# buggyyang/CDC_compression

Measured on AMD Instinct MI355X. Metric: decoded images/sec at 256x256, 500-step x-param, higher is better.
Workload: dtype f32 (f16x2 split products)

## Files before the change

cdc_compression_amd/csrc/conv_args.h:

```cpp
#pragma once
#include <stdint.h>

namespace cdc {

constexpr int kWaveSize = 64;
constexpr int kXS = 20;

struct ConvArgs {
    const float *src0, *src1;
    long long src0_bs, src1_bs;
    int uf_c, uf_pad;
    unsigned uf_magic;
    int C0, Cin;
    int H, W;
    const float *ln_mean, *ln_rstd;
    const float *ln_g, *ln_b;
    const float *wp;
    long long w_bs, w_zs;
    const unsigned short *wsp;
    long long wsp_zs;
    long long wsp_bs;
    float acc_scale;
    int tg;
    int ipw, B;
// ... 17 lines not shown
    float relu_slope;
    const float *shift;
    int shift_bs;
    const float *resid;
    long long resid_bs, resid_cs;
    const float *res3_w, *res3_x;
    long long res3_bs;
    float *stat_mean, *stat_rstd;
    int ksplit, nzz;
    int xcd_remap;
    int zfold;
    long long out_ks;
    void *out_pf;
    long long pf_bs, pf_ps;
    int pf_ys, pf_xs, pf_zoff[4];
    int pf_only;
    int *fault;
#ifdef CDC_TIMELINE
    unsigned long long *tl;
#endif
};

struct PfArgs {
    const void *src0, *src1;
    long long src0_bs, src1_bs;
    int C0, Cin;
    int H, W;
    const void *w;
    long long w_zs;
    int KH, KW, nz;
    int stride;
    int tz;
    int pad_y[4], pad_x[4];
    int nchunk, COP, Cout;
    float acc_scale;
    int ring;
    int n_iter;
    float *out;
    long long out_bs, out_cs;
    int out_ys, out_xs, out_zoff[4];
    void *out_pf;
    long long pf_bs, pf_ps;
    int pf_ys, pf_xs, pf_zoff[4];
    int Ho, Wo;
    int lognbw, tiles_x, tiles_y, B;
    int xcd_remap;
    const float *bias, *pre_add, *ep_g, *ep_b;
    int pre_c4;
    float eps;
    int relu;
    float relu_slope;
    const float *shift;
    int shift_bs;
    const float *resid;
    long long resid_bs, resid_cs;
    const float *resid1;
    long long resid1_bs;
    int resid_c0;
    const void *resid_pf;
    long long rpf_bs, rpf_ps;
    int rpf_ys, rpf_zoff;
    float *stat_mean, *stat_rstd;
    const float *res3_w, *res3_x;
    long long res3_bs;
    const float *x0, *x1;
    long long x0_bs, x1_bs;
    const float *pre_mean, *pre_rstd;
    long long w_bs;
    int lin;
    int dbg;
    int *fault;
#ifdef CDC_TIMELINE
    unsigned long long *tl;
#endif
};

constexpr int kPfXS = 12;

struct ConvPlan {
    int MB, NPW, WN;
    int groups;
    int KC, nchunk;
    int lognbw, tiles_x, tiles_y, PH, PW;
    int xvec, xshift[4];
    size_t lds_bytes;
    int lnmode;
    int tg;
    int ipw;
    int ksplit = 1;
    int xu = 1;
    int arith = 0;
    int split;
};

}
```

cdc_compression_amd/csrc/conv_inst_p.hip:

```cpp
#include <algorithm>
#include <map>
#include <string>
#include <vector>
#include <stdlib.h>

#include "cdc_internal.h"
#include "conv_pf_kernel.h"

namespace cdc {

template <int KH, int KW>
static pf_kernel_fn pf_lookup_k(int MB, int NPW, int WM, int WP) {
    if (MB == 2 && NPW == 2 && WM == 1 && WP == 4) return conv_pf_kernel<2, 2, 1, 4, KH, KW>;
    if (MB == 2 && NPW == 2 && WM == 2 && WP == 2) return conv_pf_kernel<2, 2, 2, 2, KH, KW>;
    if (MB == 2 && NPW == 2 && WM == 2 && WP == 4) return conv_pf_kernel<2, 2, 2, 4, KH, KW>;
    if (MB == 3 && NPW == 2 && WM == 2 && WP == 4) return conv_pf_kernel<3, 2, 2, 4, KH, KW>;
    if (MB == 3 && NPW == 1 && WM == 2 && WP == 4 && KH == 3) return conv_pf_kernel<3, 1, 2, 4, KH, KW>;
    if (MB == 2 && NPW == 2 && WM == 4 && WP == 2) return conv_pf_kernel<2, 2, 4, 2, KH, KW>;
    return nullptr;
}
static pf_kernel_fn pf_lookup_s2(int MB, int NPW, int WM, int WP) {
    if (MB == 2 && NPW == 1 && WM == 1 && WP == 4) return conv_pf_kernel<2, 1, 1, 4, 3, 3, 2>;
    if (MB == 2 && NPW == 2 && WM == 2 && WP == 2) return conv_pf_kernel<2, 2, 2, 2, 3, 3, 2>;
    if (MB == 3 && NPW == 1 && WM == 2 && WP == 4) return conv_pf_kernel<3, 1, 2, 4, 3, 3, 2>;
// ... 102 lines not shown
            if (COPT != s.Cout) continue;
            const int ring = pf_ring(c.MB, c.NPW, c.WM, c.WP, 2, 2, 1, 4);
            const int tps = pf_tps(c.MB, c.NPW, c.WM, c.WP, 2, 2, 1, 4);
            const int S = (s.Cin / 16) * 16 / tps;
            if (!ring || S < ring - 1) continue;
            const double wgs = (double)((s.Wo + 31) / 32) * ((s.Ho + TH - 1) / TH) * s.B;
            const double min_wgs = dev_env("CDC_PF_TZ_MIN_WGS") ? atof(dev_env("CDC_PF_TZ_MIN_WGS")) : 128.0;
            if (wgs < min_wgs) continue;
            best = COPT;
            const size_t patch = (size_t)2 * pf_patch_units(c.NPW, c.WP, 2, 2, 1, 4) * 16, wst = (size_t)tps * pf_rows(c.MB, 4 * c.NPW) * COPT * 16;
            p->MB = c.MB; p->NPW = c.NPW; p->WM = c.WM; p->WP = c.WP;
            p->ring = ring;
            p->tiles_x = (s.Wo + 31) / 32; p->tiles_y = (s.Ho + TH - 1) / TH;
            p->groups = 1;
            p->lds_bytes = std::max(patch + ring * wst, sizeof(float) * (size_t)(4 * COPT + 2 * c.WM * c.WP * 4 * c.NPW * 32));
            break;
        }
        return best >= 0;
    }
    for (const PfCand &c : kCands) {
        if (f[0] && (c.MB != f[0] || c.NPW != f[1] || c.WM != f[2] || c.WP != f[3])) continue;
        const int COPT = c.WM * c.MB * 32, NW = c.WM * c.WP;
        if (s.Cout % COPT) continue;
        if (s.need_all_cout && COPT != s.Cout) continue;
        if (!pf_lookup(c.MB, c.NPW, c.WM, c.WP, s.KH, s.KW)) continue;
        const int TH = c.WP * c.NPW, PH = TH + s.KH - 1, PW = 32 + s.KW - 1;
        const int xsw = (4 * PH * PW + 63) / 64;
        if (xsw > 2 * kPfXS) continue;
        const int taps = s.KH * s.KW, npb = taps == 1 ? 3 : 2;
        const size_t patch = (size_t)npb * xsw * 64 * 16, wst = (size_t)pf_rows(c.MB, c.NPW) * COPT * 16;
        const int ring = pf_ring(c.MB, c.NPW, c.WM, c.WP, s.KH, s.KW);
        if (!ring) continue;
        const int S = (s.Cin / 16) * taps;
        if (S < ring - 1) continue;
        const double wgs = (double)((s.Wo + 31) / 32) * ((s.Ho + TH - 1) / TH) * s.B * (s.Cout / COPT) * s.nz;
        const double min_waves = dev_env("CDC_PF_MIN_WAVES") ? atof(dev_env("CDC_PF_MIN_WAVES")) : 256.0;
        if (wgs * NW < min_waves) continue;
        if (c.MB == 3 && c.NPW == 1 && wgs < 128.0) continue;
        const double fill = std::min(1.0, wgs * NW / 2048.0);
        const double reads = (3.0 * c.MB + 2.0 * c.NPW) / (3.0 * c.MB * c.NPW);
        const double score = fill * (1.0 - 0.35 * reads) * (s.Cout / COPT > 1 ? 0.9 : 1.0);
        if (score > best) {
            best = score;
            p->MB = c.MB; p->NPW = c.NPW; p->WM = c.WM; p->WP = c.WP;
            p->ring = ring;
            p->tiles_x = (s.Wo + 31) / 32; p->tiles_y = (s.Ho + TH - 1) / TH;
            p->groups = s.Cout / COPT;
            p->lds_bytes = std::max(patch + ring * wst, sizeof(float) * (size_t)(4 * COPT + 2 * c.WM * c.WP * c.NPW * 32));
        }
    }
    return best >= 0;
}

hipError_t pf_launch(PfArgs a, const PfPlan &p, int B, int nz, hipStream_t st) {
    if (p.pf3_epv) return pf3_launch(a, p, B, st);
    pf_kernel_fn fn = pf_lookup(p.MB, p.NPW, p.WM, p.WP, a.KH, a.KW, a.stride == 2 ? 2 : 1, a.tz == 4 ? 4 : 1);
    if (!fn) return hipErrorInvalidValue;
    if (a.tz == 4) nz = 1;
    a.lognbw = 5;
    a.dbg = 0;
    a.tiles_x = p.tiles_x; a.tiles_y = p.tiles_y; a.B = B; a.ring = p.ring;
    if (hipError_t e = ensure_dynamic_lds((const void *)fn, p.lds_bytes); e != hipSuccess) return e;
    dim3 grid((unsigned)(p.tiles_x * p.tiles_y * B), (unsigned)p.groups, (unsigned)nz);
    a.xcd_remap = (grid.x % 8 == 0 && grid.x >= 64) ? 1 : 0;
#ifdef CDC_TIMELINE
    static unsigned long long *tl_dev = nullptr;
    static std::map<std::string, int> seen;
    const size_t tl_wgs = (size_t)grid.x * grid.y * grid.z;
    char key[96];
    snprintf(key, sizeof key, "%dx%d s%d tz%d %d->%d out %dx%d", a.KH, a.KW, a.stride == 2 ? 2 : 1, a.tz == 4 ? 4 : 1, a.Cin, a.Cout, a.Ho, a.Wo);
    a.tl = nullptr;
    if (tl_wgs <= (1u << 18) && seen[key]++ < 3) {
        if (!tl_dev) hipMalloc(&tl_dev, sizeof(unsigned long long) * 16 * (1u << 18));
        hipMemsetAsync(tl_dev, 0, sizeof(unsigned long long) * 16 * tl_wgs, st);
        a.tl = tl_dev;
    }
#endif
    hipLaunchKernelGGL(fn, grid, dim3(64 * p.WM * p.WP), p.lds_bytes, st, a);
#ifdef CDC_TIMELINE
    if (a.tl) {
        hipStreamSynchronize(st);
        std::vector<unsigned long long> h(16 * tl_wgs);
        hipMemcpy(h.data(), tl_dev, h.size() * 8, hipMemcpyDeviceToHost);
        unsigned long long t0 = ~0ull, t1 = 0;
        double cat[7] = {0}, life = 0;
        std::map<unsigned long long, int> per_cu;
        std::vector<unsigned long long> starts;
        for (size_t w = 0; w < tl_wgs; ++w) {
            const unsigned long long *r = &h[w * 16];
            for (int c = 0; c < 7; ++c) cat[c] += (double)r[c];
            t0 = std::min(t0, r[7]); t1 = std::max(t1, r[8]);
            life += (double)(r[8] - r[7]);
            per_cu[(r[10] & 0xf) << 32 | (r[9] & 0xffff00)]++;
            starts.push_back(r[7]);
        }
        std::sort(starts.begin(), starts.end());
        int cu_min = 1 << 30, cu_max = 0;
        for (auto &kv : per_cu) { cu_min = std::min(cu_min, kv.second); cu_max = std::max(cu_max, kv.second); }
        static const char *names[7] = {"setup", "prologue issue", "prologue wait", "main loop", "epilogue parameters", "epilogue arithmetic", "epilogue stores"};
        fprintf(stderr, "[pf timeline] conv %s: %zu workgroups x %d threads, lds %zu; kernel span %llu cycles, mean workgroup life %.0f; %zu CUs used, %d .. %d workgroups per CU;"
                        " start of the median / last workgroup at %llu / %llu; per workgroup (wave 0):", key, tl_wgs, 64 * p.WM * p.WP, p.lds_bytes, t1 - t0, life / tl_wgs,
                per_cu.size(), cu_min, cu_max, starts[starts.size() / 2] - t0, starts.back() - t0);
        for (int c = 0; c < 7; ++c) fprintf(stderr, "  %s %.0f", names[c], cat[c] / tl_wgs);
        fprintf(stderr, "\n");
    }
#endif
    return hipGetLastError();
}

__global__ void __launch_bounds__(256) pf_pack_kernel(const float *src, long long src_bs, uint4 *dst, long long dst_bs,
                                                      int C, int H, int W) {
    const int b = blockIdx.y;
    const long long n = (long long)(C / 8) * H * W;
    const long long i = (long long)blockIdx.x * 256 + threadIdx.x;
    if (i >= n) return;
    const int x = (int)(i % W);
    const long long t = i / W;
    const int y = (int)(t % H), g = (int)(t / H);
    const float *sp = src + (size_t)b * src_bs + ((size_t)g * 8 * H + y) * W + x;
    f16x8 hv, lv;
#pragma unroll
    for (int q = 0; q < 8; ++q) {
        _Float16 h, l;
        split2h(sp[(size_t)q * H * W], h, l);
        hv[q] = h; lv[q] = l;
    }
    const long long ps = (long long)(H + 2) * (W + 2);
    uint4 *dp = dst + (size_t)b * dst_bs + (long long)g * 2 * ps + (long long)(y + 1) * (W + 2) + x + 1;
    dp[0] = __builtin_bit_cast(uint4, hv);
    dp[ps] = __builtin_bit_cast(uint4, lv);
}

hipError_t pf_pack_launch(const float *src, long long src_bs, void *dst, long long dst_bs, int C, int H, int W, int B,
                          hipStream_t st) {
    const long long n = (long long)(C / 8) * H * W;
    dim3 grid((unsigned)((n + 255) / 256), (unsigned)B);
    hipLaunchKernelGGL(pf_pack_kernel, grid, dim3(256), 0, st, src, src_bs, reinterpret_cast<uint4 *>(dst), dst_bs, C, H, W);
    return hipGetLastError();
}

__global__ void __launch_bounds__(256) c4_pack_kernel(const float *src, long long src_bs, float4 *dst, int C, long long HW) {
    const int b = blockIdx.y;
    const long long n = (long long)(C / 4) * HW;
    const long long i = (long long)blockIdx.x * 256 + threadIdx.x;
    if (i >= n) return;
    const long long pix = i % HW, g = i / HW;
    const float *sp = src + (size_t)b * src_bs + (size_t)g * 4 * HW + pix;
    dst[(size_t)b * n + i] = make_float4(sp[0], sp[HW], sp[2 * HW], sp[3 * HW]);
}

hipError_t c4_pack_launch(const float *src, long long src_bs, float *dst, int C, long long HW, int B, hipStream_t st) {
    const long long n = (long long)(C / 4) * HW;
    dim3 grid((unsigned)((n + 255) / 256), (unsigned)B);
    hipLaunchKernelGGL(c4_pack_kernel, grid, dim3(256), 0, st, src, src_bs, reinterpret_cast<float4 *>(dst), C, HW);
// ... 28 lines not shown
```

cdc_compression_amd/csrc/conv_pf_kernel.h:

```cpp
#pragma once
#include <type_traits>

#include "conv_split_kernel.h"

namespace cdc {


#ifndef CDC_DMA_WAIT_MARGIN
#define CDC_DMA_WAIT_MARGIN 1
#endif
#ifdef CDC_DMA_WAIT_ALL
constexpr int kVmWaitMask = 0;
#else
constexpr int kVmWaitMask = ~0;
#endif
template <int N> __device__ __forceinline__ void vm_wait() { asm volatile("s_waitcnt vmcnt(%0)" ::"n"(N & kVmWaitMask) : "memory"); }

__device__ __forceinline__ void dma16(unsigned voff, const void *sbase, unsigned lds_byte) {
    asm volatile("s_mov_b32 m0, %2\n\ts_nop 0\n\tglobal_load_lds_dwordx4 %0, %1" ::"v"(voff), "s"(sbase), "s"(lds_byte)
                 : "memory");
}

template <int N, class F> __device__ __forceinline__ void static_for(F &&f) {
    if constexpr (N > 0) {
        static_for<N - 1>(f);
        f(std::integral_constant<int, N - 1>{});
    }
}

__host__ __device__ constexpr bool pf_acc2(int MB, int NPW) { return MB * NPW <= 4; }
__host__ __device__ constexpr int pf_rows(int MB, int NPW) { return pf_acc2(MB, NPW) ? 4 : 6; }
__host__ __device__ constexpr int pf_patch_units(int NPW, int WP, int KH, int KW, int STR = 1, int TZ = 1) {
    return TZ == 4 ? ((4 * (WP * NPW + 2) * 34 + 63) / 64) * 64 : ((4 * ((WP * NPW - 1) * STR + KH) * (31 * STR + KW) + 63) / 64) * 64;
}
__host__ __device__ constexpr int pf_uf_stage_floats(int NPW, int WP) { return ((3 * (WP * NPW + 6) * 38 + 63) / 64) * 64; }
#ifndef CDC_PF_S2_NPB
#define CDC_PF_S2_NPB 2
#endif
__host__ __device__ constexpr int pf_patch_bufs(int KH, int KW, int STR = 1) { return STR == 2 ? CDC_PF_S2_NPB : (KH * KW == 1 ? 3 : 2); }
__host__ __device__ constexpr int pf_ring_tps(int MB, int NPW, int WM, int WP, int KH, int KW, int STR, int tps, int TZ = 1) {
    const size_t budget = ((WM * WP == 8 || STR == 2) ? 156 * 1024 : 80 * 1024) - ((KH == 7 && KW == 1) ? pf_uf_stage_floats(NPW, WP) * 4 : 0);
    const size_t patch = (size_t)pf_patch_bufs(KH, KW, STR) * pf_patch_units(NPW, WP, KH, KW, STR, TZ) * 16;
    const size_t wst = (size_t)tps * pf_rows(MB, TZ * NPW) * WM * MB * 32 * 16;
#ifndef CDC_PF_RING_MAX
#define CDC_PF_RING_MAX 5
#endif
    for (int r = CDC_PF_RING_MAX; r >= 3; --r)
        if (patch + r * wst <= budget) return r;
    return 0;
}
#ifndef CDC_PF_S2_TPS
#define CDC_PF_S2_TPS 3
#endif
#ifndef CDC_PF_TZ_MINB
#define CDC_PF_TZ_MINB 2
#endif
#ifndef CDC_PF_TZ_TPS
#define CDC_PF_TZ_TPS 2
#endif
__host__ __device__ constexpr int pf_tps(int MB, int NPW, int WM, int WP, int KH, int KW, int STR = 1, int TZ = 1) {
    if (TZ == 4) return (CDC_PF_TZ_TPS > 1 && pf_ring_tps(MB, NPW, WM, WP, KH, KW, STR, CDC_PF_TZ_TPS, TZ) >= 3) ? CDC_PF_TZ_TPS : 1;
    return (STR == 2 && CDC_PF_S2_TPS > 1 && pf_ring_tps(MB, NPW, WM, WP, KH, KW, STR, CDC_PF_S2_TPS) >= 3) ? CDC_PF_S2_TPS : 1;
}
__host__ __device__ constexpr int pf_ring(int MB, int NPW, int WM, int WP, int KH, int KW, int STR = 1, int TZ = 1) {
    return pf_ring_tps(MB, NPW, WM, WP, KH, KW, STR, pf_tps(MB, NPW, WM, WP, KH, KW, STR, TZ), TZ);
}
#ifndef CDC_PF_ABLATE
#define CDC_PF_ABLATE 0
#endif

template <int MB, int NPW, int WM, int WP, int KH, int KW, int STR = 1, int TZ = 1, int UF = 0>
__global__ void __launch_bounds__(64 * WM * WP, (KH == 1 && KW == 7) ? 3 : STR == 2 ? 1 : ((WM * WP == 8 || MB * NPW * TZ <= 4 || (TZ == 4 && MB * NPW <= 2 && CDC_PF_TZ_MINB == 2)) ? 2 : 1)) conv_pf_kernel(const PfArgs P) {
    constexpr int NW = WM * WP, NT = 64 * NW, COPT = WM * MB * 32;
    static_assert(COPT % 64 == 0 || COPT == 32, "a weight DMA instruction (64 units) must stay inside one (plane, k-half) row");
    static_assert(TZ == 1 || (TZ == 4 && KH == 2 && KW == 2 && STR == 1), "fused phases: the 2x2 phase form of the 4x4 transposed convolution");
    constexpr int NB = TZ * NPW;
    constexpr bool ACC2 = pf_acc2(MB, NB);
    constexpr int NPL = ACC2 ? 2 : 3, ROWS = 2 * NPL;
    constexpr int WI = (ROWS * COPT + 63) / 64;
    constexpr int NWV = NW - 2;
    constexpr int NWW = (WI + NWV - 1) / NWV;
    constexpr int TAPZ = KH * KW, TAPS = TAPZ * TZ;
    constexpr int NBW = 32, NBH = 1;
    constexpr int TH = WP * NPW * NBH;
    constexpr int PH = TZ == 4 ? TH + 2 : (TH - 1) * STR + KH, PW = TZ == 4 ? NBW + 2 : (NBW - 1) * STR + KW, PLANE = PH * PW;
    constexpr int NE = (PW + 1) / 2;
    constexpr int NX = 4 * PLANE;
    constexpr int XSW = (NX + 63) / 64;
    constexpr int KX = (XSW + 1) / 2;
    constexpr int PST = XSW * 64;
    constexpr int NPB = pf_patch_bufs(KH, KW, STR), LA = NPB - 1;
    constexpr int TPS = pf_tps(MB, NPW, WM, WP, KH, KW, STR, TZ);
    static_assert(TAPZ % TPS == 0, "a weight stage is a whole number of taps of one chunk (and of one phase)");
    constexpr int SPC = TAPS / TPS;
    constexpr int TAPW = ROWS * COPT;
    constexpr int WST = TPS * TAPW;
    static_assert(UF != 0 || KX <= (STR == 2 ? 20 : kPfXS), "patch too large for two patch waves");
    static_assert(UF == 0 || (UF == 3 && KH == 7 && KW == 1 && STR == 1 && TZ == 1 && NPB == 2), "UF: the 7x1 form of the first layer");
    static_assert(STR == 1 || (STR == 2 && KH == 3 && KW == 3), "stride 2 is the 3x3 Downsample form");
    extern __shared__ __attribute__((aligned(16))) uint4 smem_u[];
#ifdef CDC_TIMELINE
    unsigned long long tl_acc[7] = {0, 0, 0, 0, 0, 0, 0}, tl_last = __builtin_readcyclecounter();
    const unsigned long long tl_start = tl_last;
#define PFTL(c) do { const unsigned long long n_ = __builtin_readcyclecounter(); tl_acc[c] += n_ - tl_last; tl_last = n_; } while (0)
#define PFTL_END() do { if (P.tl && threadIdx.x == 0) { unsigned long long *r_ = P.tl + 16 * ((size_t)blockIdx.x + (size_t)gridDim.x * (blockIdx.y + (size_t)gridDim.y * blockIdx.z)); \
        for (int c_ = 0; c_ < 7; ++c_) r_[c_] = tl_acc[c_]; r_[7] = tl_start; r_[8] = __builtin_readcyclecounter(); \
        unsigned hw_; asm volatile("s_getreg_b32 %0, hwreg(HW_REG_HW_ID)" : "=s"(hw_)); r_[9] = hw_; \
        unsigned xcc_; asm volatile("s_getreg_b32 %0, hwreg(HW_REG_XCC_ID)" : "=s"(xcc_)); r_[10] = xcc_; } } while (0)
#else
#define PFTL(c) do { } while (0)
#define PFTL_END() do { } while (0)
#endif
    const int tid = threadIdx.x, lane = tid & 63;
    const int wave = __builtin_amdgcn_readfirstlane(tid >> 6);
    const int wm = wave / WP, wp = wave % WP;
    const bool patch_wave = wave >= NWV;
    const int pwi = wave - NWV;
    const int z = blockIdx.z, cog = blockIdx.y;
// ... 128 lines not shown
#pragma unroll
                for (int m = 0; m < MB; ++m)
#pragma unroll
                    for (int n = 0; n < NPW; ++n)
                        acc[m][q0 + n] = __builtin_amdgcn_mfma_f32_32x32x16_f16(A[PA[term] % NPL][m], Bv[PB[term]][n], acc[m][q0 + n], 0, 0, 0);
            }
        }
    };

    PFTL(0);
    if constexpr (UF != 0) {
        if (!patch_wave)
            for (int q = 0; q < R - 1 && q < S; ++q) issue_w();
        constexpr int XW = NBW + 6;
        float *xs = reinterpret_cast<float *>(smem_u + NPB * PST + R * WST);
        {
            constexpr int NS = (UF * PH * XW + NT - 1) / NT;
            float sv[NS];
#pragma unroll
            for (int k = 0; k < NS; ++k) {
                const int i = tid + k * NT;
                const int ci = i / (PH * XW), rem = i - ci * (PH * XW), r = rem / XW, cc = rem - r * XW;
                const int iy = oy0 - 3 + r, ix = ox0 - 3 + cc;
                sv[k] = (i < UF * PH * XW && iy >= 0 && iy < P.H && ix >= 0 && ix < P.W) ? P.x0[(size_t)b * P.x0_bs + ((size_t)ci * P.H + iy) * P.W + ix] : 0.f;
            }
#pragma unroll
            for (int k = 0; k < NS; ++k)
                if (tid + k * NT < UF * PH * XW) xs[tid + k * NT] = sv[k];
        }
        __syncthreads();
        for (int px = tid; px < PLANE; px += NT) {
            const int r = px / PW, c = px - r * PW;
            _Float16 hq[32], lq[32];
#pragma unroll
            for (int ch = 0; ch < 32; ++ch) {
                if (ch < 7 * UF) split2h(xs[((ch % UF) * PH + r) * XW + c + ch / UF], hq[ch], lq[ch]);
                else { hq[ch] = (_Float16)0.f; lq[ch] = (_Float16)0.f; }
            }
#pragma unroll
            for (int q = 0; q < 4; ++q) {
                f16x8 hv, lv;
#pragma unroll
                for (int t = 0; t < 8; ++t) { hv[t] = hq[8 * q + t]; lv[t] = lq[8 * q + t]; }
                uint4 *pbuf = smem_u + (q >> 1) * PST + ((q & 1) * 2) * PLANE + px;
                pbuf[0] = __builtin_bit_cast(uint4, hv);
                pbuf[PLANE] = __builtin_bit_cast(uint4, lv);
            }
        }
    } else if (patch_wave) {
        for (int c = 0; c < LA && c < P.nchunk; ++c) issue_patch(c, std::integral_constant<int, -1>{});
    } else {
        for (int q = 0; q < R - 1 && q < S; ++q) issue_w();
    }
    PFTL(1);
    dma_wait();
    __builtin_amdgcn_s_barrier();
    PFTL(2);
    OpsA A0, A1;
    OpsB B0, B1;
    fetch(std::integral_constant<int, 0>{}, b_base, a_base, A0, B0);
    int rem = S - 1;
    int sn = 0;
    auto tap = [&](auto tc, auto tailc, int chunk, const uint4 *xb_cur, const uint4 *xb_nxt, OpsA &Ac, OpsB &Bc, OpsA &An,
                   OpsB &Bn) {
        constexpr int t = decltype(tc)::value;
        constexpr bool TAIL = decltype(tailc)::value;
        constexpr bool SEND = (t % TPS) == TPS - 1;
        if constexpr (!SEND) {
            if (!(CDC_PF_ABLATE && (P.dbg & 64)))
                fetch(std::integral_constant<int, t + 1>{}, xb_cur, a_base + sn * WST + ((t + 1) % TPS) * TAPW, An, Bn);
            if (patch_wave) {
                if constexpr (t < ISSUE_TAPS)
                    if (UF == 0 && chunk + LA < P.nchunk && !(CDC_PF_ABLATE && (P.dbg & 2))) issue_patch(chunk + LA, tc);
            }
        } else {
        if (!(TAIL && t == TAPS - 1) || rem > 0) {
            if (++sn == R) sn = 0;
            if (CDC_PF_ABLATE && (P.dbg & 8)) {
            } else if (patch_wave) {
                if constexpr (t == TAPS - 1) {
                    if (LA == 2 && TAPS > 1 && chunk + LA < P.nchunk) vm_wait<XSW / 2>();
                    else dma_wait();
                }
            } else if (!TAIL || rem >= R - 2) {
                vm_wait<(R - 3 - (R >= 5 ? CDC_DMA_WAIT_MARGIN : 0)) * NWW * TPS>();
            } else {
                dma_wait();
            }
            if (!(CDC_PF_ABLATE && (P.dbg & 4))) __builtin_amdgcn_s_barrier();
            const uint4 *wa = a_base + sn * WST;
            if (CDC_PF_ABLATE && (P.dbg & 64)) {
            } else if constexpr (t == TAPS - 1) fetch(std::integral_constant<int, 0>{}, xb_nxt, wa, An, Bn);
            else fetch(std::integral_constant<int, t + 1>{}, xb_cur, wa, An, Bn);
            if (patch_wave) {
                if constexpr (t < ISSUE_TAPS)
                    if (UF == 0 && chunk + LA < P.nchunk && !(CDC_PF_ABLATE && (P.dbg & 2))) issue_patch(chunk + LA, tc);
            } else if ((!TAIL || rem >= R - 1) && !(CDC_PF_ABLATE && (P.dbg & 1))) {
                issue_w();
            }
        }
        --rem;
        }
        __builtin_amdgcn_s_setprio(2);
        if (!(CDC_PF_ABLATE && (P.dbg & 32))) mma(Ac, Bc, std::integral_constant<int, t / TAPZ>{});
        __builtin_amdgcn_s_setprio(0);
    };
    int pbc = 0;
    auto chunk_body = [&](auto parc, auto tailc, int chunk) {
        constexpr int par0 = decltype(parc)::value;
        int pbn = pbc + 1;
        if (pbn == NPB) pbn = 0;
        const uint4 *xb_cur = b_base + pbc * PST, *xb_nxt = b_base + pbn * PST;
        static_for<TAPS>([&](auto tc) {
            constexpr int t = decltype(tc)::value;
            if constexpr (((par0 + t) & 1) == 0) tap(tc, tailc, chunk, xb_cur, xb_nxt, A0, B0, A1, B1);
            else tap(tc, tailc, chunk, xb_cur, xb_nxt, A1, B1, A0, B0);
        });
        pbc = pbn;
    };
    using P0 = std::integral_constant<int, 0>;
    using P1 = std::integral_constant<int, 1>;
    const int n_main = max(0, min(P.nchunk - 1, (S - R + 1) / SPC));
    if constexpr ((TAPS & 1) == 0) {
        int chunk = 0;
        for (; chunk < n_main; ++chunk) chunk_body(P0{}, std::false_type{}, chunk);
        for (; chunk < P.nchunk; ++chunk) chunk_body(P0{}, std::true_type{}, chunk);
    } else {
        int chunk = 0;
        for (; chunk + 1 < n_main; chunk += 2) {
            chunk_body(P0{}, std::false_type{}, chunk);
            chunk_body(P1{}, std::false_type{}, chunk + 1);
        }
        for (; chunk + 1 < P.nchunk; chunk += 2) {
            chunk_body(P0{}, std::true_type{}, chunk);
            chunk_body(P1{}, std::true_type{}, chunk + 1);
        }
        if (chunk < P.nchunk) chunk_body(P0{}, std::true_type{}, chunk);
    }

    __builtin_amdgcn_s_barrier();
    PFTL(3);
    if (CDC_PF_ABLATE && (P.dbg & 256)) { PFTL_END(); return; }
    float *ep = reinterpret_cast<float *>(smem_u);
    float *red = ep + 4 * COPT;
    for (int i = tid; i < COPT; i += NT) {
        const int co = cog * COPT + i;
        const bool ok = co < P.Cout;
        ep[i] = (ok && P.bias) ? P.bias[co] : 0.f;
        ep[COPT + i] = (ok && P.ep_g) ? P.ep_g[co] : 0.f;
        ep[2 * COPT + i] = (ok && P.ep_b) ? P.ep_b[co] : 0.f;
        ep[3 * COPT + i] = (ok && P.shift) ? P.shift[(size_t)b * P.shift_bs + co] : 0.f;
    }
    __syncthreads();
    PFTL(4);
    const float inv_c = 1.0f / (float)P.Cout;
    const int cobase = cog * COPT + wm * MB * 32;
    const float *epl = ep + wm * MB * 32 + 4 * half;
    const bool ch_ok = cobase + MB * 32 <= P.Cout || COPT == 32;
    const int nvalid = P.Cout - cobase;
    if constexpr (TZ == 4) {
        if (!P.pre_add && !P.resid && !P.resid_pf && !P.res3_w && !P.relu && !P.shift && !P.stat_mean && (WM == 1 || !P.ep_g)) {
            static_assert(!ACC2, "fused phases: one accumulator set");
#pragma unroll
            for (int py = 0; py < 2; ++py)
#pragma unroll
                for (int n = 0; n < NPW; ++n) {
                    const int q0 = (py * 2) * NPW + n, q1 = q0 + NPW;
                    const int oy = oy0 + (wp * NPW + n) * NBH + pr, ox = ox0 + pc;
                    const bool valid = (oy < P.Ho) && (ox < P.Wo) && ch_ok;
                    int eo = 0;
                    asm volatile("" : "+v"(eo));
                    const float *eq = epl + eo;
#pragma unroll
                    for (int m = 0; m < MB; ++m)
#pragma unroll
                        for (int r = 0; r < 16; ++r) {
                            const float bi = eq[m * 32 + (r & 3) + 8 * (r >> 2)];
                            acc[m][q0][r] = acc[m][q0][r] * P.acc_scale + bi;
                            acc[m][q1][r] = acc[m][q1][r] * P.acc_scale + bi;
                        }
                    if constexpr (WM == 1) {
                        if (P.ep_g) {
                            float mean[2], rinv[2];
#pragma unroll
                            for (int i = 0; i < 2; ++i) {
                                const int q = i ? q1 : q0;
                                float sm = 0.f;
#pragma unroll
                                for (int m = 0; m < MB; ++m)
#pragma unroll
                                    for (int r = 0; r < 16; ++r) sm += acc[m][q][r];
                                sm += __shfl_xor(sm, 32);
                                mean[i] = sm * inv_c;
                                float sq = 0.f;
#pragma unroll
                                for (int m = 0; m < MB; ++m)
#pragma unroll
                                    for (int r = 0; r < 16; ++r) { const float d = acc[m][q][r] - mean[i]; sq += d * d; }
                                sq += __shfl_xor(sq, 32);
                                if (P.fault && !(sq < 3.0e38f)) *P.fault = 1;
                                rinv[i] = 1.0f / sqrtf(sq * inv_c + P.eps);
                            }
#pragma unroll
                            for (int m = 0; m < MB; ++m)
#pragma unroll
                                for (int r = 0; r < 16; ++r) {
// ... 9 lines not shown
#pragma unroll
                        for (int m = 0; m < MB; ++m)
#pragma unroll
                            for (int r = 0; r < 16; ++r) sa += fabsf(acc[m][q0][r]) + fabsf(acc[m][q1][r]);
                        if (!(sa < 3.0e38f)) *P.fault = 1;
                    }
                    if (valid && !(CDC_PF_ABLATE && (P.dbg & 16))) {
                        if (P.out) {
                            float *op = P.out + (size_t)b * P.out_bs + (unsigned)(oy * P.out_ys + ox * P.out_xs + P.out_zoff[py * 2]) + (size_t)(cobase + 4 * half) * P.out_cs;
#pragma unroll
                            for (int m = 0; m < MB; ++m)
#pragma unroll
                                for (int r = 0; r < 16; ++r)
                                    *reinterpret_cast<float2 *>(op + (size_t)(m * 32 + (r & 3) + 8 * (r >> 2)) * P.out_cs) = make_float2(acc[m][q0][r], acc[m][q1][r]);
                        }
                        if (P.out_pf) {
                            const long long u0 = (long long)b * P.pf_bs + (long long)oy * P.pf_ys + (long long)ox * P.pf_xs + P.pf_zoff[py * 2] + half;
#pragma unroll
                            for (int m = 0; m < MB; ++m)
#pragma unroll
                                for (int g = 0; g < 4; ++g) {
                                    _Float16 h0[4], l0[4], h1[4], l1[4];
#pragma unroll
                                    for (int i = 0; i < 4; ++i) {
                                        split2h(acc[m][q0][g * 4 + i], h0[i], l0[i]);
                                        split2h(acc[m][q1][g * 4 + i], h1[i], l1[i]);
                                    }
                                    const f16x4 hv0 = {h0[0], h0[1], h0[2], h0[3]}, lv0 = {l0[0], l0[1], l0[2], l0[3]};
                                    const f16x4 hv1 = {h1[0], h1[1], h1[2], h1[3]}, lv1 = {l1[0], l1[1], l1[2], l1[3]};
                                    const uint2 a0 = __builtin_bit_cast(uint2, hv0), a1 = __builtin_bit_cast(uint2, hv1);
                                    const uint2 c0 = __builtin_bit_cast(uint2, lv0), c1 = __builtin_bit_cast(uint2, lv1);
                                    const uint2 sh = half ? a0 : a1, sl = half ? c0 : c1;
                                    uint2 rh, rl;
                                    rh.x = __shfl_xor(sh.x, 32); rh.y = __shfl_xor(sh.y, 32);
                                    rl.x = __shfl_xor(sl.x, 32); rl.y = __shfl_xor(sl.y, 32);
                                    const uint4 uh = half ? make_uint4(rh.x, rh.y, a1.x, a1.y) : make_uint4(a0.x, a0.y, rh.x, rh.y);
                                    const uint4 ul = half ? make_uint4(rl.x, rl.y, c1.x, c1.y) : make_uint4(c0.x, c0.y, rl.x, rl.y);
                                    uint4 *pu = reinterpret_cast<uint4 *>(P.out_pf) + u0 + (long long)((cobase >> 3) + m * 4 + g) * 2 * P.pf_ps;
                                    pu[0] = uh;
                                    pu[P.pf_ps] = ul;
                                }
                        }
                    }
                    __builtin_amdgcn_sched_barrier(0);
                }
            PFTL(6);
            PFTL_END();
            return;
        }
    }
    float mean_v[NB], rinv_v[NB];
    bool valid_v[NB];
    unsigned pix_v[NB];
#pragma unroll
    for (int n = 0; n < NB; ++n) {
        const int oy = oy0 + (wp * NPW + n % NPW) * NBH + pr, ox = ox0 + pc;
        const int zn = TZ == 4 ? n / NPW : z;
        valid_v[n] = (oy < P.Ho) && (ox < P.Wo) && ch_ok;
        pix_v[n] = (unsigned)(oy * P.out_ys + ox * P.out_xs + P.out_zoff[zn]);
        const float *eq = epl;
#pragma unroll
        for (int m = 0; m < MB; ++m)
#pragma unroll
            for (int r = 0; r < 16; ++r)
                acc[m][n][r] = (ACC2 ? acc[m][n][r] + acc2[ACC2 ? m : 0][ACC2 ? n : 0][r] * (1.0f / 2048.0f) : acc[m][n][r]) * P.acc_scale +
                               eq[m * 32 + (r & 3) + 8 * (r >> 2)];
        if (P.pre_add && P.pre_c4 && valid_v[n]) {
            const size_t hw = (size_t)P.Ho * P.Wo;
            const float4 *p4 = reinterpret_cast<const float4 *>(P.pre_add) + ((size_t)b * (P.Cout >> 2) + (cobase >> 2) + half) * hw + (size_t)oy * P.Wo + ox;
#pragma unroll
            for (int m = 0; m < MB; ++m)
#pragma unroll
                for (int g = 0; g < 4; ++g) {
                    const float4 v = p4[(size_t)(m * 8 + 2 * g) * hw];
                    acc[m][n][4 * g] += v.x; acc[m][n][4 * g + 1] += v.y; acc[m][n][4 * g + 2] += v.z; acc[m][n][4 * g + 3] += v.w;
                }
        } else if (P.pre_add && valid_v[n]) {
            const float *pp = P.pre_add + (size_t)b * P.out_bs + pix_v[n] + (size_t)(cobase + 4 * half) * P.out_cs;
#pragma unroll
            for (int m = 0; m < MB; ++m)
#pragma unroll
                for (int r = 0; r < 16; ++r) acc[m][n][r] += pp[(size_t)(m * 32 + (r & 3) + 8 * (r >> 2)) * P.out_cs];
        }
    }
    auto chan_stats = [&](float *mean_o, float *rinv_o) {
        const int slot = (wp * NB) * 32 + j;
        float part[NB];
#pragma unroll
        for (int n = 0; n < NB; ++n) {
            float sm = 0.f;
#pragma unroll
            for (int m = 0; m < MB; ++m)
#pragma unroll
                for (int r = 0; r < 16; ++r) sm += acc[m][n][r];
            sm += __shfl_xor(sm, 32);
            part[n] = sm;
        }
        if constexpr (WM > 1) {
            __syncthreads();
#pragma unroll
            for (int n = 0; n < NB; ++n)
                if (half == 0) red[wm * (WP * NB * 32) + slot + n * 32] = part[n];
            __syncthreads();
#pragma unroll
            for (int n = 0; n < NB; ++n) {
                float sm = 0.f;
#pragma unroll
                for (int q = 0; q < WM; ++q) sm += red[q * (WP * NB * 32) + slot + n * 32];
                part[n] = sm;
            }
        }
#pragma unroll
        for (int n = 0; n < NB; ++n) {
            mean_o[n] = part[n] * inv_c;
            float sq = 0.f;
#pragma unroll
            for (int m = 0; m < MB; ++m)
#pragma unroll
                for (int r = 0; r < 16; ++r) { const float d = acc[m][n][r] - mean_o[n]; sq += d * d; }
            sq += __shfl_xor(sq, 32);
            part[n] = sq;
        }
        if constexpr (WM > 1) {
            float *red2 = red + WM * (WP * NB * 32);
#pragma unroll
            for (int n = 0; n < NB; ++n)
                if (half == 0) red2[wm * (WP * NB * 32) + slot + n * 32] = part[n];
            __syncthreads();
#pragma unroll
            for (int n = 0; n < NB; ++n) {
                float sq = 0.f;
#pragma unroll
                for (int q = 0; q < WM; ++q) sq += red2[q * (WP * NB * 32) + slot + n * 32];
                part[n] = sq;
            }
        }
#pragma unroll
        for (int n = 0; n < NB; ++n) {
            if (P.fault && !(part[n] < 3.0e38f)) *P.fault = 1;
            rinv_o[n] = 1.0f / sqrtf(part[n] * inv_c + P.eps);
        }
    };
    if (P.ep_g) {
        chan_stats(mean_v, rinv_v);
#pragma unroll
        for (int n = 0; n < NB; ++n) {
            const float *eq = epl;
#pragma unroll
            for (int m = 0; m < MB; ++m)
#pragma unroll
                for (int r = 0; r < 16; ++r) {
                    const int ci = m * 32 + (r & 3) + 8 * (r >> 2);
                    acc[m][n][r] = (acc[m][n][r] - mean_v[n]) * rinv_v[n] * eq[COPT + ci] + eq[2 * COPT + ci];
                }
        }
    } else if (P.fault) {
#pragma unroll
        for (int n = 0; n < NB; ++n) {
            float s = 0.f;
#pragma unroll
            for (int m = 0; m < MB; ++m)
#pragma unroll
                for (int r = 0; r < 16; ++r) s += fabsf(acc[m][n][r]);
            if (!(s < 3.0e38f)) *P.fault = 1;
        }
    }
#pragma unroll
    for (int n = 0; n < NB; ++n) {
        if (P.relu) {
#pragma unroll
            for (int m = 0; m < MB; ++m)
#pragma unroll
                for (int r = 0; r < 16; ++r) acc[m][n][r] = fmaxf(acc[m][n][r], P.relu_slope * acc[m][n][r]);
        }
        if (P.shift) {
            const float *eq = epl;
#pragma unroll
            for (int m = 0; m < MB; ++m)
#pragma unroll
                for (int r = 0; r < 16; ++r) acc[m][n][r] += eq[3 * COPT + m * 32 + (r & 3) + 8 * (r >> 2)];
        }
        if (P.resid_pf && valid_v[n]) {
            const int oy = oy0 + (wp * NPW + n % NPW) * NBH + pr, ox = ox0 + pc;
            const uint2 *up = reinterpret_cast<const uint2 *>(reinterpret_cast<const uint4 *>(P.resid_pf) + (long long)b * P.rpf_bs + (long long)(cobase >> 3) * 2 * P.rpf_ps +
                                                              (long long)oy * P.rpf_ys + ox + P.rpf_zoff) + half;
#pragma unroll
            for (int m = 0; m < MB; ++m)
#pragma unroll
                for (int g = 0; g < 4; ++g) {
                    const uint2 hu = up[(long long)((m * 4 + g) * 2) * P.rpf_ps * 2], lu = up[(long long)((m * 4 + g) * 2 + 1) * P.rpf_ps * 2];
                    const f16x4 hv = __builtin_bit_cast(f16x4, hu), lv = __builtin_bit_cast(f16x4, lu);
#pragma unroll
                    for (int i = 0; i < 4; ++i) acc[m][n][g * 4 + i] += __builtin_fmaf((float)lv[i], 1.0f / 2048.0f, (float)hv[i]);
                }
        } else if (P.resid && valid_v[n]) {
            const float *rp = (P.resid1 && cobase >= P.resid_c0)
                                  ? P.resid1 + (size_t)b * P.resid1_bs + pix_v[n] + (size_t)(cobase - P.resid_c0 + 4 * half) * P.resid_cs
                                  : P.resid + (size_t)b * P.resid_bs + pix_v[n] + (size_t)(cobase + 4 * half) * P.resid_cs;
#pragma unroll
            for (int m = 0; m < MB; ++m)
#pragma unroll
                for (int r = 0; r < 16; ++r) acc[m][n][r] += rp[(size_t)(m * 32 + (r & 3) + 8 * (r >> 2)) * P.resid_cs];
        }
    }
    if (P.res3_w) {
        const size_t hw = (size_t)P.Ho * P.Wo;
#pragma unroll
        for (int n = 0; n < NB; ++n) {
            const int oy = oy0 + (wp * NPW + n % NPW) * NBH + pr, ox = ox0 + pc;
            const float *xp = P.res3_x + (size_t)b * P.res3_bs + (size_t)oy * P.Wo + ox;
            const float x0 = valid_v[n] ? xp[0] : 0.f, x1 = valid_v[n] ? xp[hw] : 0.f, x2 = valid_v[n] ? xp[2 * hw] : 0.f;
#pragma unroll
            for (int m = 0; m < MB; ++m)
#pragma unroll
                for (int r = 0; r < 16; ++r) {
                    const int co = cobase + m * 32 + (r & 3) + 8 * (r >> 2) + 4 * half;
                    acc[m][n][r] += P.res3_w[co] * x0 + P.res3_w[(size_t)P.COP + co] * x1 + P.res3_w[2 * (size_t)P.COP + co] * x2;
                }
        }
    }
    if (P.stat_mean) {
        chan_stats(mean_v, rinv_v);
#pragma unroll
        for (int n = 0; n < NB; ++n)
            if (valid_v[n] && half == 0 && wm == 0) {
                P.stat_mean[(size_t)b * P.out_cs + pix_v[n]] = mean_v[n];
                P.stat_rstd[(size_t)b * P.out_cs + pix_v[n]] = rinv_v[n];
            }
    }
    PFTL(5);
    if constexpr (TZ == 4) {
#pragma unroll
        for (int py = 0; py < 2; ++py)
#pragma unroll
            for (int n = 0; n < NPW; ++n) {
                const int q0 = (py * 2) * NPW + n, q1 = q0 + NPW;
                if (!valid_v[q0] || (CDC_PF_ABLATE && (P.dbg & 16))) continue;
                if (P.out) {
                    float *op = P.out + (size_t)b * P.out_bs + pix_v[q0] + (size_t)(cobase + 4 * half) * P.out_cs;
#pragma unroll
                    for (int m = 0; m < MB; ++m)
#pragma unroll
                        for (int r = 0; r < 16; ++r)
                            *reinterpret_cast<float2 *>(op + (size_t)(m * 32 + (r & 3) + 8 * (r >> 2)) * P.out_cs) = make_float2(acc[m][q0][r], acc[m][q1][r]);
                }
                if (P.out_pf) {
                    const int oy = oy0 + (wp * NPW + n) * NBH + pr, ox = ox0 + pc;
                    const long long u0 = (long long)b * P.pf_bs + (long long)oy * P.pf_ys + (long long)ox * P.pf_xs + P.pf_zoff[py * 2] + half;
#pragma unroll
                    for (int m = 0; m < MB; ++m)
#pragma unroll
                        for (int g = 0; g < 4; ++g) {
                            _Float16 h0[4], l0[4], h1[4], l1[4];
#pragma unroll
                            for (int i = 0; i < 4; ++i) {
                                split2h(acc[m][q0][g * 4 + i], h0[i], l0[i]);
                                split2h(acc[m][q1][g * 4 + i], h1[i], l1[i]);
                            }
                            const f16x4 hv0 = {h0[0], h0[1], h0[2], h0[3]}, lv0 = {l0[0], l0[1], l0[2], l0[3]};
                            const f16x4 hv1 = {h1[0], h1[1], h1[2], h1[3]}, lv1 = {l1[0], l1[1], l1[2], l1[3]};
                            const uint2 a0 = __builtin_bit_cast(uint2, hv0), a1 = __builtin_bit_cast(uint2, hv1);
                            const uint2 c0 = __builtin_bit_cast(uint2, lv0), c1 = __builtin_bit_cast(uint2, lv1);
                            const uint2 sh = half ? a0 : a1, sl = half ? c0 : c1;
                            uint2 rh, rl;
                            rh.x = __shfl_xor(sh.x, 32); rh.y = __shfl_xor(sh.y, 32);
                            rl.x = __shfl_xor(sl.x, 32); rl.y = __shfl_xor(sl.y, 32);
                            const uint4 uh = half ? make_uint4(rh.x, rh.y, a1.x, a1.y) : make_uint4(a0.x, a0.y, rh.x, rh.y);
                            const uint4 ul = half ? make_uint4(rl.x, rl.y, c1.x, c1.y) : make_uint4(c0.x, c0.y, rl.x, rl.y);
                            uint4 *pu = reinterpret_cast<uint4 *>(P.out_pf) + u0 + (long long)((cobase >> 3) + m * 4 + g) * 2 * P.pf_ps;
                            pu[0] = uh;
                            pu[P.pf_ps] = ul;
                        }
                }
            }
        PFTL(6);
        PFTL_END();
        return;
    }
#pragma unroll
    for (int n = 0; n < NB; ++n) {
        if (!valid_v[n] || (CDC_PF_ABLATE && (P.dbg & 16))) continue;
        if (P.out) {
            float *op = P.out + (size_t)b * P.out_bs + pix_v[n] + (size_t)(cobase + 4 * half) * P.out_cs;
#pragma unroll
            for (int m = 0; m < MB; ++m)
#pragma unroll
                for (int r = 0; r < 16; ++r) {
                    const int ci = m * 32 + (r & 3) + 8 * (r >> 2);
                    if (COPT != 32 || ci + 4 * half < nvalid) op[(size_t)ci * P.out_cs] = acc[m][n][r];
                }
        }
        if (P.out_pf) {
            const int oy = oy0 + (wp * NPW + n % NPW) * NBH + pr, ox = ox0 + pc;
            const long long u0 = (long long)b * P.pf_bs + (long long)oy * P.pf_ys + (long long)ox * P.pf_xs + P.pf_zoff[TZ == 4 ? n / NPW : z];
#pragma unroll
            for (int m = 0; m < MB; ++m)
                pf_store_block(reinterpret_cast<uint4 *>(P.out_pf), u0 + (long long)((cobase >> 3) + m * 4) * 2 * P.pf_ps, P.pf_ps, half, acc[m][n]);
        }
    }
    PFTL(6);
    PFTL_END();
}

typedef void (*pf_kernel_fn)(const PfArgs);

}
```

Baseline: 5.428.

## Prefetch epilogue params early, use permlane32 swap, add 16-byte LDS-transposed epilogue I/O

Epilogue parameters (bias, gain, beta, shift) now load into a separate LDS region before the main loop, when it fits, so their global latency overlaps the prologue instead of stalling after it. Cross-half reductions use the gfx950 permlane32_swap builtin in place of a shuffle. An optional path stages the epilogue's residual and pre-add reads and its output writes through per-wave LDS transposes so global accesses become 16-byte row vectors. That path sits behind CDC_PF_EPI16, which defaults to 0. The early prefetch raises LDS use, which may reduce occupancy.

```diff
diff --git a/cdc_compression_amd/csrc/conv_args.h b/cdc_compression_amd/csrc/conv_args.h
--- a/cdc_compression_amd/csrc/conv_args.h
+++ b/cdc_compression_amd/csrc/conv_args.h
@@ -93,6 +93,7 @@
     float relu_slope;
     const float *shift;
     int shift_bs;
+    int io16;
     const float *resid;
     long long resid_bs, resid_cs;
     const float *resid1;
diff --git a/cdc_compression_amd/csrc/conv_inst_p.hip b/cdc_compression_amd/csrc/conv_inst_p.hip
--- a/cdc_compression_amd/csrc/conv_inst_p.hip
+++ b/cdc_compression_amd/csrc/conv_inst_p.hip
@@ -178,15 +178,34 @@
     return best >= 0;
 }
 
+static bool pf_rows16(const PfArgs &a, const PfPlan &p, int nz) {
+    if (a.tz == 4 || dev_env("CDC_PF_IO4")) return false;
+    if (a.Wo % 32 || a.Ho % (p.WP * p.NPW) || a.Cout % (p.MB * 32)) return false;
+    const auto al = [](const void *q, long long bs, long long cs) { return ((size_t)q & 15) == 0 && bs % 4 == 0 && cs % 4 == 0; };
+    if (a.out_xs != 1 || a.out_ys % 4) return false;
+    for (int z = 0; z < nz && z < 4; ++z)
+        if (a.out_zoff[z] % 4) return false;
+    if (a.out && !al(a.out, a.out_bs, a.out_cs)) return false;
+    if (a.pre_add && !a.pre_c4 && !al(a.pre_add, a.out_bs, a.out_cs)) return false;
+    if (a.resid && !a.resid_pf) {
+        if (!al(a.resid, a.resid_bs, a.resid_cs)) return false;
+        if (a.resid1 && !al(a.resid1, a.resid1_bs, a.resid_cs)) return false;
+    }
+    return true;
+}
+
 hipError_t pf_launch(PfArgs a, const PfPlan &p, int B, int nz, hipStream_t st) {
     if (p.pf3_epv) return pf3_launch(a, p, B, st);
-    pf_kernel_fn fn = pf_lookup(p.MB, p.NPW, p.WM, p.WP, a.KH, a.KW, a.stride == 2 ? 2 : 1, a.tz == 4 ? 4 : 1);
+    const int STR = a.stride == 2 ? 2 : 1, TZ = a.tz == 4 ? 4 : 1;
+    pf_kernel_fn fn = pf_lookup(p.MB, p.NPW, p.WM, p.WP, a.KH, a.KW, STR, TZ);
     if (!fn) return hipErrorInvalidValue;
     if (a.tz == 4) nz = 1;
     a.lognbw = 5;
     a.dbg = 0;
     a.tiles_x = p.tiles_x; a.tiles_y = p.tiles_y; a.B = B; a.ring = p.ring;
-    if (hipError_t e = ensure_dynamic_lds((const void *)fn, p.lds_bytes); e != hipSuccess) return e;
+    a.io16 = pf_rows16(a, p, nz) ? 1 : 0;
+    const size_t lds_bytes = pf_lds_bytes(p.lds_bytes, p.MB, p.NPW, p.WM, p.WP, a.KH, a.KW, STR, TZ);
+    if (hipError_t e = ensure_dynamic_lds((const void *)fn, lds_bytes); e != hipSuccess) return e;
     dim3 grid((unsigned)(p.tiles_x * p.tiles_y * B), (unsigned)p.groups, (unsigned)nz);
     a.xcd_remap = (grid.x % 8 == 0 && grid.x >= 64) ? 1 : 0;
 #ifdef CDC_TIMELINE
@@ -202,7 +221,7 @@
         a.tl = tl_dev;
     }
 #endif
-    hipLaunchKernelGGL(fn, grid, dim3(64 * p.WM * p.WP), p.lds_bytes, st, a);
+    hipLaunchKernelGGL(fn, grid, dim3(64 * p.WM * p.WP), lds_bytes, st, a);
 #ifdef CDC_TIMELINE
     if (a.tl) {
         hipStreamSynchronize(st);
@@ -225,7 +244,7 @@
         for (auto &kv : per_cu) { cu_min = std::min(cu_min, kv.second); cu_max = std::max(cu_max, kv.second); }
         static const char *names[7] = {"setup", "prologue issue", "prologue wait", "main loop", "epilogue parameters", "epilogue arithmetic", "epilogue stores"};
         fprintf(stderr, "[pf timeline] conv %s: %zu workgroups x %d threads, lds %zu; kernel span %llu cycles, mean workgroup life %.0f; %zu CUs used, %d .. %d workgroups per CU;"
-                        " start of the median / last workgroup at %llu / %llu; per workgroup (wave 0):", key, tl_wgs, 64 * p.WM * p.WP, p.lds_bytes, t1 - t0, life / tl_wgs,
+                        " start of the median / last workgroup at %llu / %llu; per workgroup (wave 0):", key, tl_wgs, 64 * p.WM * p.WP, lds_bytes, t1 - t0, life / tl_wgs,
                 per_cu.size(), cu_min, cu_max, starts[starts.size() / 2] - t0, starts.back() - t0);
         for (int c = 0; c < 7; ++c) fprintf(stderr, "  %s %.0f", names[c], cat[c] / tl_wgs);
         fprintf(stderr, "\n");
diff --git a/cdc_compression_amd/csrc/conv_pf_kernel.h b/cdc_compression_amd/csrc/conv_pf_kernel.h
--- a/cdc_compression_amd/csrc/conv_pf_kernel.h
+++ b/cdc_compression_amd/csrc/conv_pf_kernel.h
@@ -20,6 +20,26 @@
     asm volatile("s_mov_b32 m0, %2\n\ts_nop 0\n\tglobal_load_lds_dwordx4 %0, %1" ::"v"(voff), "s"(sbase), "s"(lds_byte)
                  : "memory");
 }
+
+#ifndef CDC_PF_EPI16
+#define CDC_PF_EPI16 0
+#endif
+#ifndef CDC_PF_EP_EARLY
+#define CDC_PF_EP_EARLY 1
+#endif
+#ifndef CDC_PF_SWAP32
+#define CDC_PF_SWAP32 1
+#endif
+__device__ __forceinline__ unsigned xchg32(unsigned v) {
+#if CDC_PF_SWAP32 && defined(__gfx950__) && __has_builtin(__builtin_amdgcn_permlane32_swap)
+    const auto r = __builtin_amdgcn_permlane32_swap(v, v, false, false);
+    return __lane_id() >= 32 ? r[0] : r[1];
+#else
+    return __shfl_xor(v, 32);
+#endif
+}
+typedef float pf_f4 __attribute__((ext_vector_type(4)));
+__device__ __forceinline__ float xchg32(float v) { return __builtin_bit_cast(float, xchg32(__builtin_bit_cast(unsigned, v))); }
 
 template <int N, class F> __device__ __forceinline__ void static_for(F &&f) {
     if constexpr (N > 0) {
@@ -64,6 +84,19 @@
 }
 __host__ __device__ constexpr int pf_ring(int MB, int NPW, int WM, int WP, int KH, int KW, int STR = 1, int TZ = 1) {
     return pf_ring_tps(MB, NPW, WM, WP, KH, KW, STR, pf_tps(MB, NPW, WM, WP, KH, KW, STR, TZ), TZ);
+}
+__host__ __device__ constexpr size_t pf_ops_bytes(int MB, int NPW, int WM, int WP, int KH, int KW, int STR = 1, int TZ = 1) {
+    return (size_t)pf_patch_bufs(KH, KW, STR) * pf_patch_units(NPW, WP, KH, KW, STR, TZ) * 16 +
+           (size_t)pf_ring(MB, NPW, WM, WP, KH, KW, STR, TZ) * pf_tps(MB, NPW, WM, WP, KH, KW, STR, TZ) * pf_rows(MB, TZ * NPW) * WM * MB * 32 * 16 +
+           ((KH == 7 && KW == 1) ? (size_t)pf_uf_stage_floats(NPW, WP) * 4 : 0);
+}
+__host__ __device__ constexpr bool pf_ep_early(int MB, int NPW, int WM, int WP, int KH, int KW, int STR = 1, int TZ = 1) {
+    const size_t cap = (WM * WP == 8 || STR == 2) ? 160 * 1024 : ((KH == 1 && KW == 7) ? 160 * 1024 / 3 : 80 * 1024);
+    return CDC_PF_EP_EARLY && TZ == 1 && pf_ops_bytes(MB, NPW, WM, WP, KH, KW, STR, TZ) + (size_t)16 * WM * MB * 32 <= cap;
+}
+__host__ __device__ constexpr size_t pf_lds_bytes(size_t plan_bytes, int MB, int NPW, int WM, int WP, int KH, int KW, int STR = 1, int TZ = 1) {
+    const size_t early = pf_ep_early(MB, NPW, WM, WP, KH, KW, STR, TZ) ? pf_ops_bytes(MB, NPW, WM, WP, KH, KW, STR, TZ) + (size_t)16 * WM * MB * 32 : 0;
+    return plan_bytes > early ? plan_bytes : early;
 }
 #ifndef CDC_PF_ABLATE
 #define CDC_PF_ABLATE 0
@@ -298,6 +331,21 @@
     } else {
         for (int q = 0; q < R - 1 && q < S; ++q) issue_w();
     }
+    constexpr bool EP_EARLY = pf_ep_early(MB, NPW, WM, WP, KH, KW, STR, TZ);
+    static_assert(pf_ops_bytes(MB, NPW, WM, WP, KH, KW, STR, TZ) == ((size_t)NPB * PST + (size_t)R * WST) * 16 + (UF ? (size_t)pf_uf_stage_floats(NPW, WP) * 4 : 0),
+                  "pf_ops_bytes is the kernel's own layout");
+    if constexpr (EP_EARLY) {
+        float *epw = reinterpret_cast<float *>(smem_u) + pf_ops_bytes(MB, NPW, WM, WP, KH, KW, STR, TZ) / 4;
+        for (int i = tid; i < COPT; i += NT) {
+            const int co = cog * COPT + i;
+            const bool ok = co < P.Cout;
+            epw[i] = (ok && P.bias) ? P.bias[co] : 0.f;
+            epw[COPT + i] = (ok && P.ep_g) ? P.ep_g[co] : 0.f;
+            epw[2 * COPT + i] = (ok && P.ep_b) ? P.ep_b[co] : 0.f;
+            epw[3 * COPT + i] = (ok && P.shift) ? P.shift[(size_t)b * P.shift_bs + co] : 0.f;
+        }
+        asm volatile("s_waitcnt lgkmcnt(0)" ::: "memory");
+    }
     PFTL(1);
     dma_wait();
     __builtin_amdgcn_s_barrier();
@@ -387,17 +435,22 @@
     __builtin_amdgcn_s_barrier();
     PFTL(3);
     if (CDC_PF_ABLATE && (P.dbg & 256)) { PFTL_END(); return; }
-    float *ep = reinterpret_cast<float *>(smem_u);
-    float *red = ep + 4 * COPT;
-    for (int i = tid; i < COPT; i += NT) {
-        const int co = cog * COPT + i;
-        const bool ok = co < P.Cout;
-        ep[i] = (ok && P.bias) ? P.bias[co] : 0.f;
-        ep[COPT + i] = (ok && P.ep_g) ? P.ep_g[co] : 0.f;
-        ep[2 * COPT + i] = (ok && P.ep_b) ? P.ep_b[co] : 0.f;
-        ep[3 * COPT + i] = (ok && P.shift) ? P.shift[(size_t)b * P.shift_bs + co] : 0.f;
-    }
-    __syncthreads();
+    float *red = reinterpret_cast<float *>(smem_u) + 4 * COPT;
+    constexpr bool IO16 = CDC_PF_EPI16 && TZ == 1;
+    constexpr int XR0 = 4 * COPT + 2 * WM * WP * NB * 32;
+    static_assert(!IO16 || (size_t)(XR0 + NW * 1024) * 4 <= ((size_t)NPB * PST + (size_t)R * WST) * 16, "the transposition regions fit in the operand buffers");
+    float *ep = reinterpret_cast<float *>(smem_u) + (EP_EARLY ? pf_ops_bytes(MB, NPW, WM, WP, KH, KW, STR, TZ) / 4 : 0);
+    if constexpr (!EP_EARLY) {
+        for (int i = tid; i < COPT; i += NT) {
+            const int co = cog * COPT + i;
+            const bool ok = co < P.Cout;
+            ep[i] = (ok && P.bias) ? P.bias[co] : 0.f;
+            ep[COPT + i] = (ok && P.ep_g) ? P.ep_g[co] : 0.f;
+            ep[2 * COPT + i] = (ok && P.ep_b) ? P.ep_b[co] : 0.f;
+            ep[3 * COPT + i] = (ok && P.shift) ? P.shift[(size_t)b * P.shift_bs + co] : 0.f;
+        }
+        __syncthreads();
+    }
     PFTL(4);
     const float inv_c = 1.0f / (float)P.Cout;
     const int cobase = cog * COPT + wm * MB * 32;
@@ -513,6 +566,24 @@
     float mean_v[NB], rinv_v[NB];
     bool valid_v[NB];
     unsigned pix_v[NB];
+    const bool io16 = IO16 && P.io16;
+    const int Lr = lane >> 3, Lc = lane & 7;
+    float *xr = reinterpret_cast<float *>(smem_u) + XR0 + wave * 1024;
+    auto add_rows = [&](int n, const float *src, long long cs) {
+        const float *sp = src + (size_t)Lr * cs + 4 * Lc;
+        pf_f4 rows[MB][4];
+#pragma unroll
+        for (int m = 0; m < MB; ++m)
+#pragma unroll
+            for (int k = 0; k < 4; ++k) rows[m][k] = *reinterpret_cast<const pf_f4 *>(sp + (size_t)(m * 32 + 8 * k) * cs);
+#pragma unroll
+        for (int m = 0; m < MB; ++m) {
+#pragma unroll
+            for (int k = 0; k < 4; ++k) *reinterpret_cast<pf_f4 *>(xr + (Lr + 8 * k) * 32 + Lc * 4) = rows[m][k];
+#pragma unroll
+            for (int r = 0; r < 16; ++r) acc[m][n][r] += xr[((r & 3) + 8 * (r >> 2) + 4 * half) * 32 + j];
+        }
+    };
 #pragma unroll
     for (int n = 0; n < NB; ++n) {
         const int oy = oy0 + (wp * NPW + n % NPW) * NBH + pr, ox = ox0 + pc;
@@ -537,11 +608,15 @@
                     acc[m][n][4 * g] += v.x; acc[m][n][4 * g + 1] += v.y; acc[m][n][4 * g + 2] += v.z; acc[m][n][4 * g + 3] += v.w;
                 }
         } else if (P.pre_add && valid_v[n]) {
-            const float *pp = P.pre_add + (size_t)b * P.out_bs + pix_v[n] + (size_t)(cobase + 4 * half) * P.out_cs;
-#pragma unroll
-            for (int m = 0; m < MB; ++m)
-#pragma unroll
-                for (int r = 0; r < 16; ++r) acc[m][n][r] += pp[(size_t)(m * 32 + (r & 3) + 8 * (r >> 2)) * P.out_cs];
+            if (io16) {
+                add_rows(n, P.pre_add + (size_t)b * P.out_bs + (pix_v[n] - pc) + (size_t)cobase * P.out_cs, P.out_cs);
+            } else {
+                const float *pp = P.pre_add + (size_t)b * P.out_bs + pix_v[n] + (size_t)(cobase + 4 * half) * P.out_cs;
+#pragma unroll
+                for (int m = 0; m < MB; ++m)
+#pragma unroll
+                    for (int r = 0; r < 16; ++r) acc[m][n][r] += pp[(size_t)(m * 32 + (r & 3) + 8 * (r >> 2)) * P.out_cs];
+            }
         }
     }
     auto chan_stats = [&](float *mean_o, float *rinv_o) {
@@ -554,7 +629,7 @@
             for (int m = 0; m < MB; ++m)
 #pragma unroll
                 for (int r = 0; r < 16; ++r) sm += acc[m][n][r];
-            sm += __shfl_xor(sm, 32);
+            if constexpr (TZ == 4) sm += __shfl_xor(sm, 32); else sm += xchg32(sm);
             part[n] = sm;
         }
         if constexpr (WM > 1) {
@@ -579,7 +654,7 @@
             for (int m = 0; m < MB; ++m)
 #pragma unroll
                 for (int r = 0; r < 16; ++r) { const float d = acc[m][n][r] - mean_o[n]; sq += d * d; }
-            sq += __shfl_xor(sq, 32);
+            if constexpr (TZ == 4) sq += __shfl_xor(sq, 32); else sq += xchg32(sq);
             part[n] = sq;
         }
         if constexpr (WM > 1) {
@@ -655,13 +730,19 @@
                     for (int i = 0; i < 4; ++i) acc[m][n][g * 4 + i] += __builtin_fmaf((float)lv[i], 1.0f / 2048.0f, (float)hv[i]);
                 }
         } else if (P.resid && valid_v[n]) {
-            const float *rp = (P.resid1 && cobase >= P.resid_c0)
-                                  ? P.resid1 + (size_t)b * P.resid1_bs + pix_v[n] + (size_t)(cobase - P.resid_c0 + 4 * half) * P.resid_cs
-                                  : P.resid + (size_t)b * P.resid_bs + pix_v[n] + (size_t)(cobase + 4 * half) * P.resid_cs;
-#pragma unroll
-            for (int m = 0; m < MB; ++m)
-#pragma unroll
-                for (int r = 0; r < 16; ++r) acc[m][n][r] += rp[(size_t)(m * 32 + (r & 3) + 8 * (r >> 2)) * P.resid_cs];
+            if (io16) {
+                const float *rb = (P.resid1 && cobase >= P.resid_c0) ? P.resid1 + (size_t)b * P.resid1_bs + (size_t)(cobase - P.resid_c0) * P.resid_cs
+                                                                     : P.resid + (size_t)b * P.resid_bs + (size_t)cobase * P.resid_cs;
+                add_rows(n, rb + (pix_v[n] - pc), P.resid_cs);
+            } else {
+                const float *rp = (P.resid1 && cobase >= P.resid_c0)
+                                      ? P.resid1 + (size_t)b * P.resid1_bs + pix_v[n] + (size_t)(cobase - P.resid_c0 + 4 * half) * P.resid_cs
+                                      : P.resid + (size_t)b * P.resid_bs + pix_v[n] + (size_t)(cobase + 4 * half) * P.resid_cs;
+#pragma unroll
+                for (int m = 0; m < MB; ++m)
+#pragma unroll
+                    for (int r = 0; r < 16; ++r) acc[m][n][r] += rp[(size_t)(m * 32 + (r & 3) + 8 * (r >> 2)) * P.resid_cs];
+            }
         }
     }
     if (P.res3_w) {
@@ -741,7 +822,19 @@
 #pragma unroll
     for (int n = 0; n < NB; ++n) {
         if (!valid_v[n] || (CDC_PF_ABLATE && (P.dbg & 16))) continue;
-        if (P.out) {
+        if (P.out && io16) {
+            float *op = P.out + (size_t)b * P.out_bs + (pix_v[n] - pc) + (size_t)(cobase + Lr) * P.out_cs + 4 * Lc;
+#pragma unroll
+            for (int m = 0; m < MB; ++m) {
+#pragma unroll
+                for (int r = 0; r < 16; ++r) xr[((r & 3) + 8 * (r >> 2) + 4 * half) * 32 + j] = acc[m][n][r];
+                pf_f4 rows[4];
+#pragma unroll
+                for (int k = 0; k < 4; ++k) rows[k] = *reinterpret_cast<const pf_f4 *>(xr + (Lr + 8 * k) * 32 + Lc * 4);
+#pragma unroll
+                for (int k = 0; k < 4; ++k) *reinterpret_cast<pf_f4 *>(op + (size_t)(m * 32 + 8 * k) * P.out_cs) = rows[k];
+            }
+        } else if (P.out) {
             float *op = P.out + (size_t)b * P.out_bs + pix_v[n] + (size_t)(cobase + 4 * half) * P.out_cs;
 #pragma unroll
             for (int m = 0; m < MB; ++m)
```

Result: no change. 5.435, median of 6 (+0.1%).
